# amazon-science/tubelet-transformer

Measured on AMD Instinct MI355X. Metric: clips/sec (TubeR CSN-152 AVA2.1 training step fwd+bwd+clip+AdamW, 32x256x340 clips; whole job), higher is better.
Workload: dtype bf16; 1 GPU; TubeR_CSN152_AVA21 train step, 2 clips/GPU of 3x32x256x340, dropout on, random-init name-hashed weights; global_batch=2, parallelism=dp1, launch_mode=hipgraph, lib_md5=ad1afa292c39

## Files before the change

include/tuber_hip.h:

```cpp
#ifndef TUBER_HIP_H
#define TUBER_HIP_H

#ifdef __cplusplus
extern "C" {
#endif

typedef struct ihipStream_t* hipStream_t;

typedef struct TuberClipDesc {
    long long src_off;
    int H, W;
    int y1, x1, h, w;
    int flip, jitter;
    int hue, sat, val;
    int pad_;
} TuberClipDesc;

int tuber_attn_fwd(const void* Q, const long* mq, const void* K, const long* mk, const void* V, const long* mv, void* O, const long* mo, float* lse, const void* key_padding_mask, int B, int H, int Lq, int Lk, float scale, float pdrop, const void* seed_ptr, unsigned long long salt, hipStream_t stream);

int tuber_attn_bwd(const void* Q, const long* mq, const void* K, const long* mk, const void* V, const long* mv, const void* O, const long* mo, const float* lse, const void* key_padding_mask, const void* dO, const long* mdo, void* dQ, const long* mdq, void* dK, const long* mdk, void* dV, const long* mdv, float* delta, int B, int H, int Lq, int Lk, float scale, float pdrop, const void* seed_ptr, unsigned long long salt, hipStream_t stream);

int tuber_attn_wide_fwd(const void* q, const void* kv, void* o, int NQ, int HW, int T, float pdrop, const void* seed_ptr, unsigned long long salt, hipStream_t stream);

int tuber_attn_wide_bwd(const void* q, const void* kv, const void* dO, void* dq, void* dkv, int NQ, int HW, int T, float pdrop, const void* seed_ptr, unsigned long long salt, hipStream_t stream);
// ... 206 lines not shown

int tuber_ln_bwd_dx_pays(int M, int E_, int Kin);

int tuber_ln_bwd_dx(const void* dy, long lddy, const void* dy2, long lddy2, const void* xhat, const float* rstd, const float* gamma, void* dx, void* dxd, float* partial, int M, int E_, float p, const void* seed_ptr, unsigned long long salt, const void* wt, long ldt, int Kin, void* out, const void* res, const void* cm, float alpha, const void* ga, long ldga, const void* xhat_a, const float* rstd_a, const float* gamma_a, float* partial_a, hipStream_t stream);

int tuber_lsap(const double* cost_in, int nr, int nc, long* row_ind, long* col_ind);

int tuber_stat_rows_reduced(int R);

int tuber_stat_rows_reduce(const float* st0, const float* st1, int R, int C, float* out0, float* out1, hipStream_t stream);

int tuber_bn_finalize(const float* st0, const float* st1, int R, int C, float count, const float* gamma, const float* beta, float* running_mean, float* running_var, long long* num_batches_tracked, float momentum, float eps, float* scale, float* shift, float* mean, float* invstd, hipStream_t stream);

int tuber_bn_finalize_ex(const float* st0, const float* st1, int R, int C, float count, const float* gamma, const float* beta, float* running_mean, float* running_var, long long* num_batches_tracked, float momentum, float eps, float* scale, float* shift, float* mean, float* invstd, hipStream_t stream);

int tuber_bn_count_advance(const long* table, int n, hipStream_t stream);

int tuber_bn_eval_affine(const float* gamma, const float* beta, const float* running_mean, const float* running_var, float eps, float* scale, float* shift, int C, hipStream_t stream);

int tuber_bn_eval_affine_multi(const void* table, int n, int cmax, float eps, hipStream_t stream);

int tuber_bn_frozen_affine_multi(const void* table, int n, int cmax, float eps, hipStream_t stream);

int tuber_bn_frozen_param_grads(const float* st0, const float* st1, int R, int C, const float* mean, const float* invstd, float* dgamma, float* dbeta, hipStream_t stream);

int tuber_bn_bwd_finalize(const float* st0, const float* st1, int R, int C, float count, const float* gamma, const float* mean, const float* invstd, float* cA, float* cB, float* cC, float* dgamma, float* dbeta, int accumulate, hipStream_t stream);

int tuber_block_out_fwd(const void* c4, const float* s4, const float* h4, const void* res, const float* rs, const float* rh, void* y, long M, int C, hipStream_t stream);

int tuber_block_out_fwd_mask(const void* c4, const float* s4, const float* h4, const void* res, const float* rs, const float* rh, void* y, void* ymask, long M, int C, hipStream_t stream);

int tuber_block_out_fwd_f32(const void* c4, const float* s4, const float* h4, const void* res, const float* rs, const float* rh, const float* res32, void* y, float* y32, long M, int C, hipStream_t stream);

int tuber_rowblock_count(long M, int C);

int tuber_block_out_bwd(const void* dy, const void* y, const void* c4, const void* cds, void* dz, float* st_dz, float* st_c4, float* st_ds, long M, int C, hipStream_t stream);

int tuber_bn_bwd_fa_max_rows(void);

int tuber_bn_bwd_fa_rows(long M, int C);

int tuber_bn_bwd_fa_rows_set(int kr);

int tuber_bn_bwd_fa(const float* st0, const float* st1, int R, int C, float count, const float* gamma, const float* mean, const float* invstd, float* dgamma, float* dbeta, const void* dz, const void* x, void* dx, long M, hipStream_t stream);

int tuber_bn_bwd_fa_frozen(const float* st0, const float* st1, int R, int C, const float* gamma, const float* mean, const float* invstd, float* dgamma, float* dbeta, const void* dz, void* dx, long M, hipStream_t stream);

int tuber_bn_bwd_apply(const void* dz, const void* x, const float* cA, const float* cB, const float* cC, void* dx, long M, int C, hipStream_t stream);

int tuber_layernorm_fwd(const void* x, const void* res, const float* gamma, const float* beta, void* y, long ldy, void* xhat, float* rstd, int M, int E, float eps, float p, const void* seed_ptr, unsigned long long salt, hipStream_t stream);

int tuber_layernorm_fwd_f32(const void* x, const float* x32, const void* res, const float* res32, const float* gamma, const float* beta, void* y, long ldy, float* y32, int M, int E, float eps, hipStream_t stream);

int tuber_layernorm_bwd_blocks(int M);

int tuber_layernorm_bwd(const void* dy, long lddy, const void* xhat, const float* rstd, const float* gamma, void* dx, void* dxd, float* partial, float* dgamma, float* dbeta, int accumulate, int M, int E, float p, const void* seed_ptr, unsigned long long salt, hipStream_t stream);

int tuber_reduce_rows(const float* P, float* out, int R, int C, int accumulate, hipStream_t stream);

int tuber_colsum_blocks(long M);

int tuber_colsum(const void* g, float* partial, float* out, int accumulate, long M, int C, long ld, hipStream_t stream);

int tuber_multi_reduce(const void* table, const void* blk, int nblocks, hipStream_t stream);

int tuber_multi_reduce_entry_bytes(void);

int tuber_grad_norm_clip_coef(const float* g, long n, float max_norm, float* partial, float* norm_out, int* step_ptr, hipStream_t stream);

int tuber_adamw_segment(float* p, float* g, float* exp_avg, float* exp_avg_sq, long n, const float* clip, float lr, float beta1, float beta2, float eps, float weight_decay, const int* step_ptr, int write_clipped_grad, const float* hyper, hipStream_t stream);

int tuber_scale_f32(float* x, long n, const float* coef_dev, float coef, hipStream_t stream);

int tuber_rows_dx2(const void* g, long ldg, int M, int N, int Nq, const void* wt, long ldt, int Kin, void* dx, const void* res, void* dpos, hipStream_t stream);

int tuber_stem_pool_fwd(const void* x, const float* sc, const float* sh, void* out, void* arg, int NT, int Hs, int Ws, int Hp, int Wp, hipStream_t stream);

int tuber_stem_pool_bwd_stat_rows(long positions);

int tuber_stem_pool_bwd(const void* gpool, const void* arg, const void* x, const float* sc, const float* sh, void* dz, float* st0, float* st1, int NT, int Hs, int Ws, int Hp, int Wp, hipStream_t stream);

int tuber_stem_conv_blocks(int B, int T, int H, int W);

int tuber_stem_conv_wgrad_blocks(int B, int T, int H, int W);

int tuber_stem_pack_weight(const float* W, void* Wp, hipStream_t stream);

int tuber_stem_conv_fwd(const float* clip, const void* Wp, void* out, float* st0, float* st1, int B, int T, int H, int W, hipStream_t stream);

int tuber_stem_conv_bwd_weight(const float* clip, const void* G, float* partial, float* dW, int accumulate, int B, int T, int H, int W, hipStream_t stream);

int tuber_stem_conv_bwd_weight_bn(const float* clip, const void* dz0, const void* c0, const float* cA, const float* cB, const float* cC, float* partial, float* dW, int accumulate, int B, int T, int H, int W, hipStream_t stream);

int tuber_flag_signal(unsigned* flag, hipStream_t stream);

int tuber_flag_wait(const unsigned* flag, unsigned expect, unsigned* err, hipStream_t stream);


#ifdef __cplusplus
}
#endif
#endif
```

tubelet_transformer_amd/csrc/gen_header.py:

```python
import glob
import os
import re

HERE = os.path.dirname(os.path.abspath(__file__))
ROOT = os.path.dirname(os.path.dirname(HERE))

DOC = {
    "tuber_gemm_nt_addproj": "packed attention in-projection with the positional embedding folded in: C = f(A).B^T + bias with f(A) = A + A2 for the output "
                             "columns [0, add_ncols) (q / k rows of in_proj_weight: with_pos_embed, models/transformer/transformer.py:150-159,215-240) and "
                             "f(A) = A for the v rows -- one GEMM instead of an add kernel and two GEMM launches. add_ncols % 128 == 0.",
    "tuber_bn_bwd_fa": "tuber_bn_bwd_finalize + tuber_bn_bwd_apply in ONE launch for short partial lists (layer3 / layer4 of the CSN body): every workgroup "
                       "derives the coefficients of its 128-channel strip from the R partial rows (fp64) and applies dx = cA*dz + cB*x + cC to its rows; "
                       "dgamma / dbeta accumulated by the first row chunk (NULL: frozen BatchNorm). autograd of nn.BatchNorm3d (ir_CSN_152.py:46,56,64,154).",
    "tuber_bn_bwd_fa_max_rows": "largest R tuber_bn_bwd_fa accepts.",
    "tuber_bn_frozen_affine_multi": "the FROZEN BatchNorm layers of a training-mode forward (nn.BatchNorm3d with module.training == False inside model.train(): "
                                    "F.batch_norm(training=False), models/backbones/ir_CSN_152.py:46,56,64,119,154) in ONE launch over a device table of "
                                    "{gamma, beta, running_mean, running_var, scale, shift, mean, invstd, cA, cB, cC, C} rows: scale / shift bit-identical to "
                                    "tuber_bn_eval_affine, mean = running_mean, invstd = 1 / sqrt(running_var + eps), and the backward coefficients cA = gamma * invstd, "
                                    "cB = cC = 0, so every backward kernel that takes (cA, cB, cC) runs unchanged. The running buffers are not written.",
    "tuber_bn_frozen_param_grads": "dgamma += sum dz * (x - running_mean) * invstd, dbeta += sum dz of a frozen BatchNorm whose affine parameters train (autograd of "
                                   "F.batch_norm(training=False), ir_CSN_152.py:46,56,64,119,154) from the partial rows (sum dz, sum dz*x) of the train-mode path: "
                                   "no count, no coefficient output.",
    "tuber_bn_bwd_fa_frozen": "tuber_bn_bwd_fa for a frozen BatchNorm: dx = gamma * invstd * dz in one launch (autograd of F.batch_norm(training=False), "
                              "ir_CSN_152.py:46,56,64,154); x is not an operand, the partial rows are read only for dgamma / dbeta (NULL: not at all).",
# ... 155 lines not shown
    "tuber_frames_resize": "PIL.Image.resize((nw, nh)) of every decoded frame (datasets/ava_frame.py:146-150; jhmdb_frame.py alike): Pillow's 8-bit two-pass "
                           "fixed-point bicubic (libImaging/Resample.c), packed RGB uint8 [nimg][H][W][3] -> [nimg][Ho][Wo][3], bit-exact.",
    "tuber_clip_prepare": "hflip + crop + ColorJitter + ToTensor/Normalize (datasets/video_transforms.py:69-85,20-66,333-369,308-322; pipeline "
                          "datasets/ava_frame.py:158-176) and the batch collate of utils/misc.py:279-282,367-425 in one pass: uint8 frames -> "
                          "fp32 [N][3][T][Hmax][Wmax] zero padded + bool mask [N][Hmax][Wmax]. One TuberClipDesc per clip (56 bytes: long long src_off; "
                          "int H, W, y1, x1, h, w, flip, jitter, hue, sat, val, pad).",
    "tuber_clip_desc_bytes": "sizeof(TuberClipDesc) as the library was compiled (host-side layout check).",
    "tuber_multi_reduce": "every deferred second-stage reduction of one backward pass in one launch: the weight-gradient launchers called with "
                          "accumulate = 2 (tuber_gemm_tn, tuber_dwconv_*_bwd_weight, tuber_colsum, tuber_layernorm_bwd) leave their partials in place; "
                          "table = MultiReduceEntry[] {const float* P; float* out; long n, stride; int S, mode, C, next}: out[j] += sum_s P[s*stride+j] "
                          "(mode 0 / 2: per element / per float4, s ascending; mode 1: 32-way tree; C > 0: depthwise [S][27][C] -> [C][27]; next: chained contribution to the same out); blk = int2[] (head entry, block in entry), "
                          "1024 / 4096 / 32 elements per block in mode 0 / 2 / 1. Same summation order as the immediate kernels.",
    "tuber_multi_reduce_entry_bytes": "sizeof(MultiReduceEntry) as compiled (host-side layout check).",
    "tuber_temporal_max_fwd": "nn.MaxPool3d((T,1,1)) over the T frames of the backbone features, TEMPORAL_DS_STRATEGY 'max' (models/backbone_builder.py:45-47,73): "
                              "rows (b,t,p) of E bf16 -> rows (b,p) + the uint8 index of the first maximal frame (arg may be NULL in eval).",
    "tuber_temporal_max_bwd": "backward of tuber_temporal_max_fwd: the gradient goes to the frame that held the maximum, zeros elsewhere.",
    "tuber_gemm_nt": "C[M,N] = f(A)[M,K] . B[N,K]^T on MFMA bf16. Replaces every nn.Conv3d(k=1) of the CSN bottlenecks "
                     "(models/backbones/ir_CSN_152.py:41,58,155-161), input_proj/class_proj (models/tuber_ava.py:57-58) and every "
                     "nn.Linear / packed in-projection (models/transformer/transformer.py:159-165,227-245; transformer_layers.py:81-94; "
                     "tuber_ava.py:65-71), plus their data gradients (B = W^T). amode 1 fuses relu(x*a_scale[k]+a_shift[k]) "
                     "(BatchNorm apply, ir_CSN_152.py:72-79) into the A load; gather=1 reads A rows through the strided "
                     "(n,t*st,h*ss,w*ss) map of the down_sample conv (:155-161). epi 0: +bias, +R, ReLU, bf16|fp32 out; "
                     "epi 1: bf16 out + per-column partial (sum, sum^2) rows for training-mode BatchNorm; epi 2: out = acc*[Cm*m_scale+m_shift>0] "
                     "+ partial (sum dz, sum dz*Cm) rows for BatchNorm backward (stat rows optional: with m_scale NULL it is the ReLU / ReLU+Dropout "
                     "backward mask from the saved activation). Accumulators are scaled by alpha first; epi 0 can end with Dropout(drop_p) "
                     "keyed by (seed, salt, m*N+n) -- FFN linear1 (transformer.py:160-162). K % 64 == 0.",
    "tuber_gemm_nt_cfg": "tile configuration tuber_gemm_nt uses for (M,N,K): 13 = 64x64 (two-tile prefetch), 7 = 64x128, 0 = 128x128 (plain epilogue only); 2 / 12 / 17 = rejected A/B variants, built only with -DTUBER_AB_VARIANTS.",
    "tuber_gemm_tn_tile": "output tile edge of the transpose-read weight-gradient kernel for (M, N, K): 128 (mid-M backbone shapes, N and K multiples of 128) or 64.",
    "tuber_gemm_nt_has_cfg": "1 when tuber_gemm_nt_set_cfg(cfg) names a tile configuration this library was built with.",
    "tuber_gemm_nt_stat_rows": "rows of partial statistics tuber_gemm_nt(epi 1|2) writes for (M,N).",
    "tuber_gemm_tn": "dW[N,K] (+)= sum_m G[m,N]^T . f(A)[m,K]: weight gradient of the same convs / linears (autograd of the ops above); "
                     "split over M into fp32 slabs `partial` [tuber_gemm_tn_slabs][N][K], then reduced deterministically.",
    "tuber_gemm_tn_fuses_bias": "can tuber_gemm_tn also produce the bias gradient for this shape: 0 no; 1 yes, accumulated into bias_grad[N] directly (single slab); 2 yes, bias_grad receives one partial row per slab ([tuber_gemm_tn_slabs][N], reduced by the caller).",
    "tuber_gemm_tn_slabs": "number of slabs (size of `partial` / (N*K)) tuber_gemm_tn uses.",
    "tuber_dwconv_fwd": "depthwise Conv3d(C,C,3,groups=C,stride=(st,ss,ss),padding=1) on NDHWC bf16, ResNeXtBottleneck.conv3 "
                        "(ir_CSN_152.py:48-51) with relu(bn1(.)) fused on load (sc/sh may be NULL) and bn3 partial statistics on store.",
    "tuber_dwconv_bwd_data": "input gradient of conv3 fused with the backward of relu(bn1(.)): dz = da*[x*sc+sh>0] + partial (sum dz, sum dz*x).",
    "tuber_dwconv_bwd_weight": "weight gradient of conv3 ([C][27] fp32), activation relu(bn1(x)) recomputed on load.",
    "tuber_dwconv_fwd_stat_rows": "partial-stat rows written by tuber_dwconv_fwd.",
    "tuber_dwconv_bwd_data_stat_rows": "partial-stat rows written by tuber_dwconv_bwd_data.",
    "tuber_dwconv_bwd_weight_blocks": "blocks (size of `partial` / (27*C)) used by tuber_dwconv_bwd_weight.",
    "tuber_dwconv_tile_fwd_bn": "tuber_bn_finalize + tuber_dwconv_tile_fwd in ONE launch: the training-mode BatchNorm in front of conv3 (bn1, ir_CSN_152.py:46-51) is "
                                "finalised inside the conv -- every workgroup derives scale / shift of its 64 channels from the producing conv's R partial rows "
                                "(pst0 = sum x, pst1 = sum x^2 over `count` rows; fp64 sums, the arithmetic of tuber_bn_finalize expression for expression), the first "
                                "workgroup of each channel group writes scale / shift / mean / invstd [C] and updates rmean / rvar / nbt (NULL: none). Other arguments as tuber_dwconv_tile_fwd.",
    "tuber_dwconv_tile_fwd_bn_ex": "tuber_dwconv_tile_fwd_bn with the momentum contract of tuber_bn_finalize_ex: the module's momentum as given, or (momentum < 0) "
                                   "the cumulative average of nn.BatchNorm3d(momentum=None) with nbt read, not written (tuber_bn_count_advance). "
                                   "reference: ir_CSN_152.py:46-51 under torch.optim.swa_utils.update_bn.",
    "tuber_dwconv_tile_fwd": "stride-1 conv3 (ir_CSN_152.py:48-51) with the input planes staged once per workgroup in an LDS ring (activated on the way in): "
                             "same contract as tuber_dwconv_fwd for st = ss = 1; partial-stat rows = tuber_dwconv_tile_blocks.",
    "tuber_dwconv_tile_bwd_data": "LDS-staged data gradient of the stride-1 conv3, fused with the backward of relu(bn1(.)) like tuber_dwconv_bwd_data.",
    "tuber_dwconv_tile_bwd_weight": "LDS-staged weight gradient of the stride-1 conv3 (activation recomputed while staging).",
    "tuber_dwconv_tile_blocks": "workgroups along x of the LDS-staged depthwise kernels = partial-stat rows / weight-gradient partial blocks.",
    "tuber_dwconv_tile_wgrad_blocks": "partial blocks (size of `partial` / (27*C)) of tuber_dwconv_tile_bwd_weight.",
    "tuber_dw_wgrad_reduce": "dw[c][tap] (+)= sum_r partial[r][tap][c]: second stage of the depthwise weight gradient.",
    "tuber_bn_finalize": "training-mode nn.BatchNorm3d(eps=1e-3, momentum=0.1) statistics (ir_CSN_152.py:15-16,46,56,64,119,154): partial rows -> "
                         "mean/invstd, scale=gamma*invstd, shift=beta-mean*scale, running_mean/var (unbiased) and num_batches_tracked update.",
    "tuber_bn_finalize_ex": "tuber_bn_finalize with the module's momentum as given (nn.BatchNorm3d.momentum, ir_CSN_152.py:15-16,46,56,64,119,154; "
                            "running = (1 - m) * running + m * batch, num_batches_tracked += 1). momentum < 0 selects the cumulative average of "
                            "momentum=None (torch.nn.modules.batchnorm._BatchNorm.forward): m = 1 / (n + 1) with n = *num_batches_tracked read on the device, "
                            "which this launch leaves unchanged so that every workgroup sees the same n -- tuber_bn_count_advance increments it after the forward.",
    "tuber_bn_count_advance": "num_batches_tracked += 1 (the `self.num_batches_tracked.add_(1)` of _BatchNorm.forward under momentum=None) for every BatchNorm "
                              "of a DEVICE table of n int64 counter addresses, in ONE launch: the layers finalised in cumulative mode by tuber_bn_finalize_ex / "
                              "tuber_dwconv_tile_fwd_bn_ex during the forward.",
    "tuber_stat_rows_reduce": "first stage for long partial-statistics lists (R > 512 rows: layer1): [R][C] x2 -> [tuber_stat_rows_reduced(R)][C] x2.",
    "tuber_stat_rows_reduced": "rows left by tuber_stat_rows_reduce (R itself when no first stage is needed).",
    "tuber_bn_eval_affine": "eval-mode BatchNorm3d folded to scale/shift from the running statistics.",
    "tuber_bn_bwd_finalize": "BatchNorm backward coefficients: dx = cA*dz + cB*x + cC, dgamma = sum dz*xhat, dbeta = sum dz.",
    "tuber_bn_bwd_apply": "dx = cA*dz + cB*x + cC (BatchNorm backward apply), bf16 [M,C].",
    "tuber_block_out_fwd": "bottleneck join y = relu(bn4(c4) + shortcut) (ir_CSN_152.py:81-90); shortcut = res or bn_ds(res) when rs/rh given.",
    "tuber_block_out_bwd": "backward of the join: dz = dy*[y>0] and the partial statistics of bn4 (and of the down_sample BN).",
    "tuber_rowblock_count": "partial-stat rows written by the row-blocked reduce kernels for M rows.",
    "tuber_layernorm_fwd": "y = LayerNorm(Dropout_p(x) (+ res)) over E in {256, 2048}, eps 1e-5 (nn.LayerNorm, transformer.py:163-167,229-247,116-123; "
                           "transformer_layers.py:84,91,96,437-445); saves xhat (bf16) and rstd for backward.",
    "tuber_layernorm_bwd": "backward of tuber_layernorm_fwd: dx (gradient of res), dxd (gradient of x through the regenerated dropout mask) and dgamma/dbeta via block partials.",
    "tuber_layernorm_bwd_blocks": "blocks used by tuber_layernorm_bwd (partial = 2*blocks*E floats).",
    "tuber_reduce_rows": "out[c] (+)= sum_r P[r][c].",
    "tuber_colsum_blocks": "row blocks (size of `partial` / C) used by tuber_colsum.",
    "tuber_colsum": "bias gradient: out[c] (+)= sum_m g[m][c] for bf16 g.",
    "tuber_gemm_nt_set_cfg": "tuning hook: force tile configuration cfg for every later tuber_gemm_nt (-1 = automatic choice).",
    "tuber_stem_conv_fwd": "stem Conv3d(3,64,(3,7,7),s=(1,2,2),p=(1,3,3)) (ir_CSN_152.py:109-115) as an implicit MFMA GEMM from the fp32 NCDHW clip to NDHWC bf16, "
                           "with the partial statistics of the following BatchNorm; Wp = tuber_stem_pack_weight(conv1.weight).",
    "tuber_stem_conv_bwd_weight": "weight gradient of the stem conv ([64][441] fp32) as an implicit MFMA GEMM (no patch matrix in HBM).",
    "tuber_stem_conv_blocks": "persistent grid size of the stem conv forward = its partial-stat rows.",
    "tuber_stem_conv_wgrad_blocks": "workgroups (= [512][64] fp32 partial slabs) of tuber_stem_conv_bwd_weight.",
    "tuber_stem_pack_weight": "conv1.weight [64][441] fp32 -> [64][512] bf16 with k' = (c,kt,kh)*8 + kw (zero padded).",
    "tuber_stem_pool_fwd": "relu(bn1(.)) + MaxPool3d((1,3,3),s=(1,2,2),p=(0,1,1)) (ir_CSN_152.py:119-122) on NDHWC bf16, C=64; saves the argmax tap.",
    "tuber_stem_pool_bwd": "backward of the pool + relu(bn1(.)): dz and the BN-backward partial statistics.",
    "tuber_stem_pool_bwd_stat_rows": "partial-stat rows written by tuber_stem_pool_bwd.",
    "tuber_attn_fwd": "softmax(scale*QK^T + key_padding_mask)[dropout] V for 32-wide heads, operands read in place through strided token maps "
                      "{ld,sL,s1,s2,B2}: row(l,b) = l*sL + (b/B2)*s1 + (b%B2)*s2. Core of nn.MultiheadAttention "
                      "(transformer.py:159,227,237; tuber_ava.py:138; transformer_layers.py:81,88) and of the hand-rolled MHA (:156-167,306-366).",
    "tuber_attn_bwd": "gradients dQ, dK, dV of tuber_attn_fwd (P recomputed from the saved log-sum-exp).",
    "tuber_attn_wide_fwd": "single-query, 256-wide-head attention of the LSTR pooling decoder (TEMPORAL_DS_STRATEGY decode; "
                           "backbone_builder.py:74-78, transformer_layers.py:156-167,306-366): q [NQ,2048], kv [rows,4096]=[k|v], T<=8 slots per pixel.",
    "tuber_attn_wide_bwd": "gradients dq [NQ,2048] and dkv [rows,4096] of tuber_attn_wide_fwd.",
    "tuber_lsap": "rectangular linear sum assignment on HOST doubles; restates scipy.optimize.linear_sum_assignment (call sites "
                  "models/detr/matcher.py:80, matcher_ucf.py:82) incl. its tie-breaking.",
    "tuber_lsap_device": "the same assignment (scipy.optimize.linear_sum_assignment semantics incl. tie-breaking; matcher.py:80, matcher_ucf.py:82) for all "
                         "(decoder layer, clip) problems at once ON THE DEVICE, one thread per problem: match[l][b][t] = query of target t.",
    "tuber_grad_norm_clip_coef": "global L2 norm of the flat gradient buffer and the clip coefficient min(1, max_norm/(norm+1e-6)), left on the device: "
                                 "torch.nn.utils.clip_grad_norm_(model.parameters(), 0.1) (utils/video_action_recognition.py:153).  A non-finite norm "
                                 "yields coefficient -1 = skip the update and leaves the step count alone: the reference stops BEFORE optimizer.step() on a "
                                 "non-finite loss (video_action_recognition.py:195-198).",
    "tuber_adamw_segment": "AdamW update (torch.optim.AdamW semantics: decoupled decay, bias correction) of one contiguous flat segment with the "
                           "clip coefficient applied to the gradient on the fly (video_action_recognition.py:154; groups train_tuber_ava.py:41-58).",
    "tuber_grad_accum": "gradient accumulation over m micro-batches (DistributedDataParallel's mean over ranks reproduced on fewer GPUs: the mean of "
                        "independent per-rank backward passes, utils/model_utils.py:47-49) over a DEVICE table of nwin [begin, end) int64 windows of the flat "
                        "fp32 gradient buffer, in ONE launch: mode 0 acc = g, mode 1 acc += g, mode 2 g = (acc + g) * scale (scale_dev[0] when given). "
                        "Fixed order: sequential fp32 sum, then one multiply. g and acc 16-byte aligned.",
    "tuber_bn_stats_copy": "snapshot (restore = 0: arena <- buffers) or restore (restore = 1: buffers <- arena) of BatchNorm running statistics "
                           "(running_mean, running_var, num_batches_tracked of nn.BatchNorm3d, models/backbones/ir_CSN_152.py:46,56,64,154) in ONE launch over a "
                           "DEVICE table of nrows {address, arena offset in 32-bit words, words} int64 rows; max_words = the largest row.",
    "tuber_scale_f32": "x *= coef: gradient averaging after the RCCL all-reduce (DistributedDataParallel's mean, utils/model_utils.py:47-49).",
    "tuber_criterion_cost": "Hungarian matching cost C = w_bbox*L1 - w_giou*GIoU - w_class*p of every decoder layer at once, [L,B,Q,Tmax] fp32 "
                            "(HungarianMatcher.forward, models/detr/matcher.py:61-76 / matcher_ucf.py:61-78; generalized_box_iou utils/box_ops.py:41-65).",
    "tuber_criterion_loss": "all loss terms of all layers and their gradients w.r.t. logits / actor logits / boxes in one launch: AVA 3-way weighted CE + "
                            "weighted BCE (models/criterion.py:42-81), JHMDB (C+1)-way CE (:237-262), L1 + GIoU box losses (:97-117).",
    "tuber_cast_f32_bf16": "fp32 -> bf16 copy (bf16 shadow of the fp32 master weights).",
    "tuber_cast_transpose": "W[R][C] fp32 -> W^T[C][ldt] bf16 (B operand of the data-gradient GEMM).",
    "tuber_rows_gather_sum": "out[(a,b,c)] = mul * sum_d in[a*sa+b*sb+c*sc+d*sd] over rows of E bf16: temporal AvgPool3d((4,1,1)) "
                             "(backbone_builder.py:44,73), its backward (broadcast), the x6 replication of src_c (tuber_ava.py:133) and its backward (sum).",
    "tuber_axpby": "out = alpha*a + beta*b (bf16): with_pos_embed adds (transformer.py:150-151), gradient accumulation.",
    "tuber_dropout": "y = keep ? x/(1-p) : 0 with a stateless hash RNG keyed by (seed, index); applying it to a gradient with the same seed is the backward.",
    "tuber_sigmoid_fwd": "boxes = sigmoid(bbox_embed(hs)) (tuber_ava.py:142).",
    "tuber_sigmoid_bwd": "dx = dy*y*(1-y).",
    "tuber_relu_mask": "dx = dy*[h>0] (ReLU backward from the saved activation; FFN and MLP hidden layers).",
    "tuber_multi_transpose_bf16": "every GEMM weight W[R][C] -> W^T[C][ldt] (bf16 shadow of the parameters -> bf16: the B operand of the data-gradient GEMMs, autograd of "
                                  "nn.Conv3d(k=1) / nn.Linear) in one launch over a device table {src_off,dst_off,R,C,ldt,tile_begin,tiles_x,pad} of 64 x 64 tiles.",
    "tuber_cast_pad_rows": "src[R][C] fp32 -> dst[R][ldd] bf16 with zero-filled pad columns (stem 441->448 taps, head gradients).",
    "tuber_rows_scatter_add": "dst[map(m)] += src[m] over the strided (n,t*st,h*ss,w*ss) row map: input gradient of a strided down_sample conv (ir_CSN_152.py:155-161).",
    "tuber_posenc": "PositionEmbeddingSine_3D (models/transformer/position_encoding.py:32-72) of a (B,T,H,W) padding mask, token-major bf16.",
}

HEADER = '''/* tuber_hip.h -- C ABI of libtuber_hip.so: the MI355X (gfx950) kernels behind the TubeR forward/backward path.
 *
 * GENERATED by tubelet_transformer_amd/csrc/gen_header.py from the extern "C" definitions in csrc/*.hip.
 *
 * The reference (amazon-science/tubelet-transformer) has no FFI or operator-plugin boundary: its hot path is stock
 * torch.nn calls (SURVEY.md section 8b).  This ABI is therefore build-defined: one launcher per kernel family, each
 * citing the reference call site(s) whose arithmetic it replaces.  Conventions:
 *   - plain pointers to DEVICE memory + explicit sizes / leading dimensions (in elements); no torch types;
 *   - activations are row-major [rows, channels] bf16 (NDHWC / token-major), master weights and statistics fp32;
 *   - the callee never allocates: outputs, saved tensors and workspaces (`partial`, `st0`, ...) are caller-owned,
 *     sized with the *_rows / *_slabs / *_blocks helper calls;
 *   - every launcher enqueues on `stream` and returns 0, a negative argument-check code (TUBER_EINVAL = -1) or the
 *     positive hipError_t of a failed launch; nothing throws across the ABI.
 */
#ifndef TUBER_HIP_H
#define TUBER_HIP_H

#ifdef __cplusplus
extern "C" {
#endif

typedef struct ihipStream_t* hipStream_t;

/* one clip of tuber_clip_prepare (device memory, 56 bytes) */
typedef struct TuberClipDesc {
    long long src_off;   /* byte offset of the clip's first frame in `frames` (uint8 [T][H][W][3]) */
    int H, W;            /* frame size */
    int y1, x1, h, w;    /* crop window in the (flipped) frame: output (y,x) reads (y1+y, x1+x) */
    int flip, jitter;    /* horizontal flip before the crop; HSV colour jitter on/off */
    int hue, sat, val;   /* ColorJitter shifts (hue in OpenCV half-degrees) */
    int pad_;
} TuberClipDesc;

# ... 50 lines not shown
```

tubelet_transformer_amd/csrc/stem_conv.hip:

```cpp
#include "common.h"

#define SW 64
#define PXW 160
#define KP 512

struct StemGeom { int B, T, H, W, Ho, Wo, tilesW, ntiles; };

struct StemTile { int wt, t, ho, b; long row0; };
__device__ __forceinline__ StemTile stem_tile(const StemGeom& g, int tile) {
    StemTile s;
    s.wt = tile % g.tilesW; int r = tile / g.tilesW;
    s.t = r % g.T; r /= g.T;
    s.ho = r % g.Ho; s.b = r / g.Ho;
    s.row0 = (((long)s.b * g.T + s.t) * g.Ho + s.ho) * g.Wo + s.wt * SW;
    return s;
}
struct StemWalk { int tile, end, step; };
__device__ __forceinline__ StemWalk stem_walk(int ntiles) {
    const int G = gridDim.x;
    if (G & 7) return StemWalk{(int)blockIdx.x, ntiles, G};
    const int chunk = (ntiles + 7) >> 3, x = blockIdx.x & 7, lo = x * chunk;
    return StemWalk{lo + (int)(blockIdx.x >> 3), min(ntiles, lo + chunk), G >> 3};
}
typedef float f32x2u __attribute__((ext_vector_type(2), aligned(4)));
typedef float f32x4u __attribute__((ext_vector_type(4), aligned(4)));

struct StemLane { int l32, half, toff, tkt, tkh; };
__device__ __forceinline__ StemLane stem_lane(const StemGeom& g) {
    StemLane L;
    const int lane = threadIdx.x & 63;
    L.l32 = lane & 31; L.half = lane >> 5;
    const int c = lane / 21, kt = (lane / 7) % 3, kh = lane % 7;
    L.tkt = kt - 1; L.tkh = kh - 3;
    L.toff = ((c * g.T + kt - 1) * g.H + kh - 3) * g.W;
    return L;
}
struct StemMeta { uint32_t kill; int sr, sl, tsr, tsl; };
__device__ __forceinline__ void stem_shift_of(int x0, int W, int& xc, int& sr, int& sl, bool& dead) {
    xc = min(max(x0, 0), W - 4);
    const int d = x0 - xc;
    dead = d >= 4 || d <= -4;
    sr = d > 0 ? 16 * min(d, 3) : 0;
    sl = d < 0 ? 16 * min(-d, 3) : 0;
}
template <int NW> struct StemRuns { int off[64 / NW], dt[64 / NW], dh[64 / NW]; };
template <int NW>
__device__ __forceinline__ StemRuns<NW> stem_runs(const StemGeom& g, int wv) {
    StemRuns<NW> R;
#pragma unroll
    for (int i = 0; i < 64 / NW; ++i) {
        const int r = wv * (64 / NW) + i;
        const int c = r / 21, kt = (r / 7) % 3, kh = r % 7;
        R.dt[i] = r < 63 ? kt - 1 : (1 << 24);
        R.dh[i] = kh - 3;
        R.off[i] = ((c * g.T + kt - 1) * g.H + kh - 3) * g.W;
    }
    return R;
}
template <int NW>
__device__ __forceinline__ void stem_fetch(const float* __restrict__ clip, const StemGeom& g, int tile, const StemLane& L,
                                           const StemRuns<NW>& R, int wv, float4 (&v)[32 / NW + 1], StemMeta& m) {
    constexpr int PAIRS = 32 / NW;
    const StemTile st = stem_tile(g, tile);
    const float* base = clip + (((long)st.b * 3 * g.T + st.t) * g.H + 2 * st.ho) * (long)g.W;
    int xc; bool dead;
    stem_shift_of(128 * st.wt - 3 + 4 * L.l32, g.W, xc, m.sr, m.sl, dead);
    m.kill = dead ? 0x7fffffffu : 0u;
#pragma unroll
    for (int p = 0; p < PAIRS; ++p) {
        int off[2]; bool ok[2];
#pragma unroll
        for (int h = 0; h < 2; ++h) {
            ok[h] = (unsigned)(st.t + R.dt[2 * p + h]) < (unsigned)g.T && (unsigned)(2 * st.ho + R.dh[2 * p + h]) < (unsigned)g.H;
            off[h] = ok[h] ? R.off[2 * p + h] : 0;
        }
        const f32x4u q = *(const f32x4u*)(base + (L.half ? off[1] : off[0]) + xc);
        v[p] = make_float4(q.x, q.y, q.z, q.w);
        if (!(L.half ? ok[1] : ok[0])) m.kill |= 1u << p;
    }
    m.tsr = m.tsl = 0;
    if (wv < 2) {
        const int lane = threadIdx.x & 63;
        int txc; bool tdead;
        stem_shift_of(128 * st.wt - 3 + 4 * (32 + wv), g.W, txc, m.tsr, m.tsl, tdead);
        const bool ok = lane < 63 && (unsigned)(st.t + L.tkt) < (unsigned)g.T && (unsigned)(2 * st.ho + L.tkh) < (unsigned)g.H;
        const f32x4u q = *(const f32x4u*)(base + (ok ? L.toff : 0) + txc);
        v[PAIRS] = make_float4(q.x, q.y, q.z, q.w);
        if (!ok || tdead) m.kill |= 1u << 31;
    }
}
__device__ __forceinline__ uint64_t stem_pack4(const float4& f, int sr, int sl, bool kill) {
    const bf16x4 b = {f2bf(f.x), f2bf(f.y), f2bf(f.z), f2bf(f.w)};
    const uint2 u = as_uint2(b);
    uint64_t w = ((uint64_t)u.y << 32) | u.x;
    w = (w >> sr) << sl;
    return kill ? 0ull : w;
}
template <int NW>
__device__ __forceinline__ void stem_park(bf16 (*P)[PXW], const float4 (&v)[32 / NW + 1], const StemMeta& m, const StemLane& L, int wv) {
    constexpr int PAIRS = 32 / NW;
#pragma unroll
    for (int p = 0; p < PAIRS; ++p)
        *(uint64_t*)&P[wv * (2 * PAIRS) + 2 * p + L.half][4 * L.l32] = stem_pack4(v[p], m.sr, m.sl, (m.kill >> p) & 1);
    if (wv < 2) *(uint64_t*)&P[threadIdx.x & 63][4 * (32 + wv)] = stem_pack4(v[PAIRS], m.tsr, m.tsl, m.kill >> 31);
}
__global__ __launch_bounds__(256, 3) void stem_conv_fwd_kernel(const float* __restrict__ clip, const bf16* __restrict__ Wp,
                                                            bf16* __restrict__ out, float* __restrict__ st0,
                                                            float* __restrict__ st1, StemGeom g) {
    __shared__ __attribute__((aligned(16))) bf16 P[2][64][PXW];
    const int lane = threadIdx.x & 63, wave = threadIdx.x >> 6;
    const int li = lane & 15, gq = lane >> 4;
    bf16x8 wf[16];
#pragma unroll
    for (int ks = 0; ks < 16; ++ks) wf[ks] = as_bf16x8(*(const uint4*)(Wp + (long)(wave * 16 + li) * KP + ks * 32 + gq * 8));
#pragma unroll
    for (int ks = 0; ks < 16; ++ks) asm volatile("" : "+v"(wf[ks]));
    float s0[4] = {0.f, 0.f, 0.f, 0.f}, s1[4] = {0.f, 0.f, 0.f, 0.f};
    float4 pre[9];
    StemMeta meta;
    const StemLane L = stem_lane(g);
    const int wv = __builtin_amdgcn_readfirstlane(wave);
    const StemRuns<4> R = stem_runs<4>(g, wv);
    const StemWalk wk = stem_walk(g.ntiles);
    int tile = wk.tile, buf = 0;
    if (tile < wk.end) {
        stem_fetch<4>(clip, g, tile, L, R, wv, pre, meta);
        stem_park<4>(P[0], pre, meta, L, wv);
    }
    __syncthreads();
    for (; tile < wk.end; tile += wk.step) {
        const int next = tile + wk.step;
        if (next < wk.end) stem_fetch<4>(clip, g, next, L, R, wv, pre, meta);
        f32x4 acc[4];
#pragma unroll
        for (int mt = 0; mt < 4; ++mt) acc[mt] = f32x4{0.f, 0.f, 0.f, 0.f};
#pragma unroll
        for (int ks = 0; ks < 16; ++ks) {
            const int run = ks * 4 + gq;
#pragma unroll
            for (int mt = 0; mt < 4; ++mt) {
                const uint32_t* p = (const uint32_t*)&P[buf][run][2 * (mt * 16 + li)];
                acc[mt] = __builtin_amdgcn_mfma_f32_16x16x32_bf16(wf[ks], as_bf16x8(make_uint4(p[0], p[1], p[2], p[3])), acc[mt], 0, 0, 0);
            }
        }
        if (next < wk.end) stem_park<4>(P[buf ^ 1], pre, meta, L, wv);
        const StemTile st = stem_tile(g, tile);
        const int wt = st.wt;
        const long row0 = st.row0;
#pragma unroll
        for (int mt = 0; mt < 4; ++mt) {
            const int w = wt * SW + mt * 16 + li;
            if (w < g.Wo) {
                bf16x4 o;
#pragma unroll
                for (int r = 0; r < 4; ++r) { o[r] = f2bf(acc[mt][r]); s0[r] += acc[mt][r]; s1[r] += acc[mt][r] * acc[mt][r]; }
                *(uint2*)(out + (row0 + mt * 16 + li) * 64 + wave * 16 + gq * 4) = as_uint2(o);
            }
        }
        __syncthreads();
        buf ^= 1;
    }
    if (st0) {
#pragma unroll
        for (int r = 0; r < 4; ++r) {
            const float a = quad16_sum(s0[r]), b2 = quad16_sum(s1[r]);
            if (li == 0) {
                st0[(long)blockIdx.x * 64 + wave * 16 + gq * 4 + r] = a;
                st1[(long)blockIdx.x * 64 + wave * 16 + gq * 4 + r] = b2;
            }
        }
    }
}

#define EOW 72
#define WG_THREADS 512
__device__ __forceinline__ void stem_park_eo(bf16 (*PE)[EOW], bf16 (*PO)[EOW], const float4 (&v)[5], const StemMeta& m, const StemLane& L, int wv) {
    auto put = [&](int r, int q, uint64_t w) {
        const uint32_t lo = (uint32_t)w, hi = (uint32_t)(w >> 32);
        *(uint32_t*)&PE[r][2 * q] = __builtin_amdgcn_perm(hi, lo, 0x05040100);
        *(uint32_t*)&PO[r][2 * q] = __builtin_amdgcn_perm(hi, lo, 0x07060302);
    };
#pragma unroll
    for (int p = 0; p < 4; ++p) put(wv * 8 + 2 * p + L.half, L.l32, stem_pack4(v[p], m.sr, m.sl, (m.kill >> p) & 1));
    if (wv < 2) put(threadIdx.x & 63, 32 + wv, stem_pack4(v[4], m.tsr, m.tsl, m.kill >> 31));
}
__device__ __forceinline__ bf16x8 stem_frag_shift(const bf16* row, int m0, int s) {
    const uint4 a = *(const uint4*)(row + m0);
    const uint2 b = *(const uint2*)(row + m0 + 8);
    uint32_t w[6] = {a.x, a.y, a.z, a.w, b.x, b.y};
    uint4 o;
    if (s & 2) { w[0] = w[1]; w[1] = w[2]; w[2] = w[3]; w[3] = w[4]; w[4] = w[5]; }
    if (s & 1) {
        o.x = __builtin_amdgcn_alignbit(w[1], w[0], 16); o.y = __builtin_amdgcn_alignbit(w[2], w[1], 16);
        o.z = __builtin_amdgcn_alignbit(w[3], w[2], 16); o.w = __builtin_amdgcn_alignbit(w[4], w[3], 16);
    } else {
        o = make_uint4(w[0], w[1], w[2], w[3]);
    }
    return as_bf16x8(o);
}

template <int MINW, bool BNG>
__global__ __launch_bounds__(WG_THREADS, MINW) void stem_conv_bwd_w_kernel(const float* __restrict__ clip, const bf16* __restrict__ G,
                                                                       const bf16* __restrict__ X, const float* __restrict__ cA,
                                                                       const float* __restrict__ cB, const float* __restrict__ cC,
                                                                       float* __restrict__ partial, StemGeom g) {
    __shared__ __attribute__((aligned(16))) bf16 PE[64][EOW];
    __shared__ __attribute__((aligned(16))) bf16 PO[64][EOW];
    __shared__ __attribute__((aligned(16))) bf16 GT[64][72];
    __shared__ __attribute__((aligned(16))) float COEF[3][64];
    if (BNG && threadIdx.x < 64) { COEF[0][threadIdx.x] = cA[threadIdx.x]; COEF[1][threadIdx.x] = cB[threadIdx.x]; COEF[2][threadIdx.x] = cC[threadIdx.x]; }
    const int lane = threadIdx.x & 63, wave = threadIdx.x >> 6;
    const int li = lane & 15, gq = lane >> 4;
    f32x4 acc[7][2];
#pragma unroll
    for (int a = 0; a < 7; ++a)
#pragma unroll
        for (int b = 0; b < 2; ++b) acc[a][b] = f32x4{0.f, 0.f, 0.f, 0.f};
    const int ci = (lane & 3) | ((lane >> 4) << 2), mi = ((lane >> 2) & 3) + 4 * wave;
    float4 pre[5];
    StemMeta meta;
    uint2 gr[2], gx[2];
    const StemLane L = stem_lane(g);
    const int wv = __builtin_amdgcn_readfirstlane(wave);
    const int nh = wv >> 2, rb = wv & 3;
    const StemRuns<8> R = stem_runs<8>(g, wv);
    auto fetch = [&](int tile) {
        stem_fetch<8>(clip, g, tile, L, R, wv, pre, meta);
        const StemTile st = stem_tile(g, tile);
#pragma unroll
        for (int j = 0; j < 2; ++j) {
            const int w = st.wt * SW + mi * 2 + j;
            gr[j] = w < g.Wo ? *(const uint2*)(G + (st.row0 + mi * 2 + j) * 64 + ci * 4) : make_uint2(0, 0);
            if (BNG) gx[j] = w < g.Wo ? *(const uint2*)(X + (st.row0 + mi * 2 + j) * 64 + ci * 4) : make_uint2(0, 0);
        }
    };
    const StemWalk wk = stem_walk(g.ntiles);
    if (wk.tile < wk.end) fetch(wk.tile);
    for (int tile = wk.tile; tile < wk.end; tile += wk.step) {
        __syncthreads();
        stem_park_eo(PE, PO, pre, meta, L, wv);
        {
            bf16x4 x0 = as_bf16x4(gr[0]), x1 = as_bf16x4(gr[1]);
            if (BNG) {
                const StemTile st = stem_tile(g, tile);
                const bool ok0 = st.wt * SW + mi * 2 < g.Wo, ok1 = st.wt * SW + mi * 2 + 1 < g.Wo;
                const float4 a = *(const float4*)&COEF[0][ci * 4], b = *(const float4*)&COEF[1][ci * 4], c = *(const float4*)&COEF[2][ci * 4];
                const float av[4] = {a.x, a.y, a.z, a.w}, bv[4] = {b.x, b.y, b.z, b.w}, cv[4] = {c.x, c.y, c.z, c.w};
                const bf16x4 y0 = as_bf16x4(gx[0]), y1 = as_bf16x4(gx[1]);
#pragma unroll
                for (int q = 0; q < 4; ++q) {
                    x0[q] = ok0 ? f2bf(fmaf(av[q], bf2f(x0[q]), fmaf(bv[q], bf2f(y0[q]), cv[q]))) : (bf16)0.f;
                    x1[q] = ok1 ? f2bf(fmaf(av[q], bf2f(x1[q]), fmaf(bv[q], bf2f(y1[q]), cv[q]))) : (bf16)0.f;
                }
            }
#pragma unroll
            for (int c = 0; c < 4; ++c) *(bf16x2*)&GT[ci * 4 + c][mi * 2] = bf16x2{x0[c], x1[c]};
        }
        if (tile + wk.step < wk.end) fetch(tile + wk.step);
        __syncthreads();
#pragma unroll
        for (int ms = 0; ms < 2; ++ms) {
            bf16x8 gb[2];
#pragma unroll
            for (int nt = 0; nt < 2; ++nt) gb[nt] = as_bf16x8(*(const uint4*)&GT[(nh * 2 + nt) * 16 + li][ms * 32 + gq * 8]);
#pragma unroll
            for (int kw = 0; kw < 7; ++kw) {
                const int kt = kw;
                const bf16* row = (kw & 1) ? &PO[rb * 16 + li][0] : &PE[rb * 16 + li][0];
                const bf16x8 pa = stem_frag_shift(row, ms * 32 + gq * 8, kw >> 1);
#pragma unroll
                for (int nt = 0; nt < 2; ++nt) acc[kt][nt] = __builtin_amdgcn_mfma_f32_16x16x32_bf16(pa, gb[nt], acc[kt][nt], 0, 0, 0);
            }
        }
    }
    float* o = partial + (long)blockIdx.x * KP * 64;
#pragma unroll
    for (int kt = 0; kt < 7; ++kt) {
        const int kw = kt;
#pragma unroll
        for (int nt = 0; nt < 2; ++nt)
#pragma unroll
            for (int r = 0; r < 4; ++r)
                o[(long)((rb * 16 + gq * 4 + r) * 8 + kw) * 64 + (nh * 2 + nt) * 16 + li] = acc[kt][nt][r];
    }
}

__global__ void stem_pack_w_kernel(const float* __restrict__ W, bf16* __restrict__ Wp) {
    const int i = blockIdx.x * blockDim.x + threadIdx.x;
    if (i >= 64 * KP) return;
    const int n = i / KP, kp = i % KP, run = kp >> 3, kw = kp & 7;
    Wp[i] = (run < 63 && kw < 7) ? f2bf(W[n * 441 + run * 7 + kw]) : (bf16)0.f;
}
__global__ __launch_bounds__(1024) void stem_wgrad_reduce_kernel(const float* __restrict__ partial, float* __restrict__ dW, int nwg, int accumulate) {
    __shared__ float red[32][33];
    const int cl = threadIdx.x & 31, rg = threadIdx.x >> 5;
    const int i = blockIdx.x * 32 + cl;
    float a = 0.f;
    for (int s = rg; s < nwg; s += 32) a += partial[(long)s * KP * 64 + i];
    red[rg][cl] = a;
    __syncthreads();
    if (rg == 0) {
        a = 0.f;
#pragma unroll
        for (int k = 0; k < 32; ++k) a += red[k][cl];
        const int kp = i / 64, n = i % 64, run = kp >> 3, kw = kp & 7;
        if (run < 63 && kw < 7) {
            float* o = dW + n * 441 + run * 7 + kw;
            *o = accumulate ? *o + a : a;
        }
    }
}

static StemGeom stem_geom(int B, int T, int H, int W) {
    StemGeom g;
    g.B = B; g.T = T; g.H = H; g.W = W;
    g.Ho = (H + 6 - 7) / 2 + 1; g.Wo = (W + 6 - 7) / 2 + 1;
    g.tilesW = (g.Wo + SW - 1) / SW;
    g.ntiles = B * T * g.Ho * g.tilesW;
    return g;
}

extern "C" {

int tuber_stem_conv_blocks(int B, int T, int H, int W) {
    constexpr int cap = 768;
    const StemGeom g = stem_geom(B, T, H, W);
    return g.ntiles < cap ? g.ntiles : cap;
}
int tuber_stem_conv_wgrad_blocks(int B, int T, int H, int W) {
    constexpr int cap = 256;
    const StemGeom g = stem_geom(B, T, H, W);
    return g.ntiles < cap ? g.ntiles : cap;
}

int tuber_stem_pack_weight(const float* W, void* Wp, hipStream_t stream) {
    hipLaunchKernelGGL(stem_pack_w_kernel, dim3(64 * KP / 256), dim3(256), 0, stream, W, (bf16*)Wp);
    TUBER_RETURN_LAUNCH();
}

int tuber_stem_conv_fwd(const float* clip, const void* Wp, void* out, float* st0, float* st1, int B, int T, int H, int W,
                        hipStream_t stream) {
    if (B <= 0 || T <= 0 || H < 7 || W < 7) return TUBER_EINVAL;
    const StemGeom g = stem_geom(B, T, H, W);
    hipLaunchKernelGGL(stem_conv_fwd_kernel, dim3(tuber_stem_conv_blocks(B, T, H, W)), dim3(256), 0, stream, clip, (const bf16*)Wp,
                       (bf16*)out, st0, st1, g);
    TUBER_RETURN_LAUNCH();
}

int tuber_stem_conv_bwd_weight(const float* clip, const void* G, float* partial, float* dW, int accumulate, int B, int T, int H, int W,
                               hipStream_t stream) {
    if (B <= 0 || T <= 0 || H < 7 || W < 7) return TUBER_EINVAL;
    const StemGeom g = stem_geom(B, T, H, W);
    const int nwg = tuber_stem_conv_wgrad_blocks(B, T, H, W);
    if (nwg > 256) hipLaunchKernelGGL((stem_conv_bwd_w_kernel<4, false>), dim3(nwg), dim3(WG_THREADS), 0, stream, clip, (const bf16*)G, nullptr, nullptr, nullptr, nullptr, partial, g);
    else hipLaunchKernelGGL((stem_conv_bwd_w_kernel<2, false>), dim3(nwg), dim3(WG_THREADS), 0, stream, clip, (const bf16*)G, nullptr, nullptr, nullptr, nullptr, partial, g);
    hipLaunchKernelGGL(stem_wgrad_reduce_kernel, dim3(KP * 64 / 32), dim3(1024), 0, stream, partial, dW, nwg, accumulate);
    TUBER_RETURN_LAUNCH();
}

int tuber_stem_conv_bwd_weight_bn(const float* clip, const void* dz0, const void* c0, const float* cA, const float* cB, const float* cC,
                                  float* partial, float* dW, int accumulate, int B, int T, int H, int W, hipStream_t stream) {
    if (B <= 0 || T <= 0 || H < 7 || W < 7 || !dz0 || !c0 || !cA || !cB || !cC) return TUBER_EINVAL;
    const StemGeom g = stem_geom(B, T, H, W);
    const int nwg = tuber_stem_conv_wgrad_blocks(B, T, H, W);
    if (nwg > 256) hipLaunchKernelGGL((stem_conv_bwd_w_kernel<4, true>), dim3(nwg), dim3(WG_THREADS), 0, stream, clip, (const bf16*)dz0, (const bf16*)c0, cA, cB, cC, partial, g);
    else hipLaunchKernelGGL((stem_conv_bwd_w_kernel<2, true>), dim3(nwg), dim3(WG_THREADS), 0, stream, clip, (const bf16*)dz0, (const bf16*)c0, cA, cB, cC, partial, g);
    hipLaunchKernelGGL(stem_wgrad_reduce_kernel, dim3(KP * 64 / 32), dim3(1024), 0, stream, partial, dW, nwg, accumulate);
    TUBER_RETURN_LAUNCH();
}

}
```

Baseline: 146.8 clips/s.

## Retile stem conv forward to 32x32 wave tiles with a smaller persistent grid

The stem conv forward now gives each wave a 32-channel by 32-column tile, so each weight fragment is reused across two column tiles. It also drops occupancy to 2 waves per SIMD and caps the grid at 512 workgroups, with unused stat rows zero-filled. Tile coordinates advance incrementally instead of using divisions each iteration, in both the forward and weight-grad kernels. The old kernel stays available behind a test hook, but the added register pressure and lower occupancy may limit the gain on a small part of the step.

Result: no change. 147.1 clips/s (median of 4 runs) (+0.2%).

```diff
diff --git a/include/tuber_hip.h b/include/tuber_hip.h
--- a/include/tuber_hip.h
+++ b/include/tuber_hip.h
@@ -312,6 +312,8 @@
 
 int tuber_stem_conv_blocks(int B, int T, int H, int W);
 
+int tuber_stem_conv_variant_set(int variant, int grid_cap);
+
 int tuber_stem_conv_wgrad_blocks(int B, int T, int H, int W);
 
 int tuber_stem_pack_weight(const float* W, void* Wp, hipStream_t stream);
diff --git a/tubelet_transformer_amd/csrc/gen_header.py b/tubelet_transformer_amd/csrc/gen_header.py
--- a/tubelet_transformer_amd/csrc/gen_header.py
+++ b/tubelet_transformer_amd/csrc/gen_header.py
@@ -261,7 +261,13 @@
     "tuber_stem_conv_fwd": "stem Conv3d(3,64,(3,7,7),s=(1,2,2),p=(1,3,3)) (ir_CSN_152.py:109-115) as an implicit MFMA GEMM from the fp32 NCDHW clip to NDHWC bf16, "
                            "with the partial statistics of the following BatchNorm; Wp = tuber_stem_pack_weight(conv1.weight).",
     "tuber_stem_conv_bwd_weight": "weight gradient of the stem conv ([64][441] fp32) as an implicit MFMA GEMM (no patch matrix in HBM).",
-    "tuber_stem_conv_blocks": "persistent grid size of the stem conv forward = its partial-stat rows.",
+    "tuber_stem_conv_blocks": "partial-statistics ROWS of the stem conv forward: st0 / st1 are [rows][64] and this is the R of the tuber_stat_rows_reduce / "
+                              "tuber_bn_finalize* call that consumes them. Not the grid: the kernel launches at most this many workgroups, workgroup b writes "
+                              "its sums to row b, and rows without an owning workgroup are written as zeros by the kernel, so all rows are defined and their sum "
+                              "is the statistic.",
+    "tuber_stem_conv_variant_set": "test hook: variant 0 = the forward's 32-channel x 32-column wave tiles (default), 1 = the 16-channel x 64-column kernel it "
+                                   "replaced (bit-identical output; kept for the parity test and A/B timing); grid_cap > 0 bounds the forward's grid so that "
+                                   "small shapes cycle the persistent loop, 0 = no bound.",
     "tuber_stem_conv_wgrad_blocks": "workgroups (= [512][64] fp32 partial slabs) of tuber_stem_conv_bwd_weight.",
     "tuber_stem_pack_weight": "conv1.weight [64][441] fp32 -> [64][512] bf16 with k' = (c,kt,kh)*8 + kw (zero padded).",
     "tuber_stem_pool_fwd": "relu(bn1(.)) + MaxPool3d((1,3,3),s=(1,2,2),p=(0,1,1)) (ir_CSN_152.py:119-122) on NDHWC bf16, C=64; saves the argmax tap.",
diff --git a/tubelet_transformer_amd/csrc/stem_conv.hip b/tubelet_transformer_amd/csrc/stem_conv.hip
--- a/tubelet_transformer_amd/csrc/stem_conv.hip
+++ b/tubelet_transformer_amd/csrc/stem_conv.hip
@@ -12,6 +12,14 @@
     s.wt = tile % g.tilesW; int r = tile / g.tilesW;
     s.t = r % g.T; r /= g.T;
     s.ho = r % g.Ho; s.b = r / g.Ho;
+    s.row0 = (((long)s.b * g.T + s.t) * g.Ho + s.ho) * g.Wo + s.wt * SW;
+    return s;
+}
+__device__ __forceinline__ StemTile stem_tile_add(const StemGeom& g, StemTile s, const StemTile& d) {
+    s.wt += d.wt; int c = s.wt >= g.tilesW; s.wt -= c ? g.tilesW : 0;
+    s.t += d.t + c; c = s.t >= g.T; s.t -= c ? g.T : 0;
+    s.ho += d.ho + c; c = s.ho >= g.Ho; s.ho -= c ? g.Ho : 0;
+    s.b += d.b + c;
     s.row0 = (((long)s.b * g.T + s.t) * g.Ho + s.ho) * g.Wo + s.wt * SW;
     return s;
 }
@@ -58,10 +66,9 @@
     return R;
 }
 template <int NW>
-__device__ __forceinline__ void stem_fetch(const float* __restrict__ clip, const StemGeom& g, int tile, const StemLane& L,
+__device__ __forceinline__ void stem_fetch(const float* __restrict__ clip, const StemGeom& g, const StemTile& st, const StemLane& L,
                                            const StemRuns<NW>& R, int wv, float4 (&v)[32 / NW + 1], StemMeta& m) {
     constexpr int PAIRS = 32 / NW;
-    const StemTile st = stem_tile(g, tile);
     const float* base = clip + (((long)st.b * 3 * g.T + st.t) * g.H + 2 * st.ho) * (long)g.W;
     int xc; bool dead;
     stem_shift_of(128 * st.wt - 3 + 4 * L.l32, g.W, xc, m.sr, m.sl, dead);
@@ -104,9 +111,13 @@
         *(uint64_t*)&P[wv * (2 * PAIRS) + 2 * p + L.half][4 * L.l32] = stem_pack4(v[p], m.sr, m.sl, (m.kill >> p) & 1);
     if (wv < 2) *(uint64_t*)&P[threadIdx.x & 63][4 * (32 + wv)] = stem_pack4(v[PAIRS], m.tsr, m.tsl, m.kill >> 31);
 }
-__global__ __launch_bounds__(256, 3) void stem_conv_fwd_kernel(const float* __restrict__ clip, const bf16* __restrict__ Wp,
-                                                            bf16* __restrict__ out, float* __restrict__ st0,
-                                                            float* __restrict__ st1, StemGeom g) {
+__device__ __forceinline__ void stem_zero_rows(float* __restrict__ st0, float* __restrict__ st1, int nrows) {
+    if (threadIdx.x < 64)
+        for (long r = (long)blockIdx.x + gridDim.x; r < nrows; r += gridDim.x) st0[r * 64 + threadIdx.x] = st1[r * 64 + threadIdx.x] = 0.f;
+}
+__global__ __launch_bounds__(256, 3) void stem_conv_fwd16_kernel(const float* __restrict__ clip, const bf16* __restrict__ Wp,
+                                                              bf16* __restrict__ out, float* __restrict__ st0,
+                                                              float* __restrict__ st1, int nrows, StemGeom g) {
     __shared__ __attribute__((aligned(16))) bf16 P[2][64][PXW];
     const int lane = threadIdx.x & 63, wave = threadIdx.x >> 6;
     const int li = lane & 15, gq = lane >> 4;
@@ -123,14 +134,17 @@
     const StemRuns<4> R = stem_runs<4>(g, wv);
     const StemWalk wk = stem_walk(g.ntiles);
     int tile = wk.tile, buf = 0;
+    const StemTile dstep = stem_tile(g, wk.step);
+    StemTile st = stem_tile(g, tile);
     if (tile < wk.end) {
-        stem_fetch<4>(clip, g, tile, L, R, wv, pre, meta);
+        stem_fetch<4>(clip, g, st, L, R, wv, pre, meta);
         stem_park<4>(P[0], pre, meta, L, wv);
     }
     __syncthreads();
     for (; tile < wk.end; tile += wk.step) {
         const int next = tile + wk.step;
-        if (next < wk.end) stem_fetch<4>(clip, g, next, L, R, wv, pre, meta);
+        const StemTile nx = stem_tile_add(g, st, dstep);
+        if (next < wk.end) stem_fetch<4>(clip, g, nx, L, R, wv, pre, meta);
         f32x4 acc[4];
 #pragma unroll
         for (int mt = 0; mt < 4; ++mt) acc[mt] = f32x4{0.f, 0.f, 0.f, 0.f};
@@ -144,7 +158,6 @@
             }
         }
         if (next < wk.end) stem_park<4>(P[buf ^ 1], pre, meta, L, wv);
-        const StemTile st = stem_tile(g, tile);
         const int wt = st.wt;
         const long row0 = st.row0;
 #pragma unroll
@@ -159,6 +172,7 @@
         }
         __syncthreads();
         buf ^= 1;
+        st = nx;
     }
     if (st0) {
 #pragma unroll
@@ -169,6 +183,110 @@
                 st1[(long)blockIdx.x * 64 + wave * 16 + gq * 4 + r] = b2;
             }
         }
+        stem_zero_rows(st0, st1, nrows);
+    }
+}
+
+template <int NM>
+__device__ __forceinline__ void stem_fwd_mma(const bf16 (*Pb)[PXW], const bf16x8 (&wf)[2][16], int gq, int col, f32x4 (&acc)[2][2]) {
+#pragma unroll
+    for (int ks = 0; ks < 16; ++ks) {
+        const int run = ks * 4 + gq;
+#pragma unroll
+        for (int mt = 0; mt < NM; ++mt) {
+            const uint32_t* p = (const uint32_t*)&Pb[run][2 * (col + mt * 16)];
+            const bf16x8 pf = as_bf16x8(make_uint4(p[0], p[1], p[2], p[3]));
+#pragma unroll
+            for (int ct = 0; ct < 2; ++ct) acc[ct][mt] = __builtin_amdgcn_mfma_f32_16x16x32_bf16(wf[ct][ks], pf, acc[ct][mt], 0, 0, 0);
+        }
+    }
+}
+__global__ __launch_bounds__(256, 2) void stem_conv_fwd_kernel(const float* __restrict__ clip, const bf16* __restrict__ Wp,
+                                                            bf16* __restrict__ out, float* __restrict__ st0,
+                                                            float* __restrict__ st1, int nrows, StemGeom g) {
+    __shared__ __attribute__((aligned(16))) bf16 P[2][64][PXW];
+    const int lane = threadIdx.x & 63, wave = threadIdx.x >> 6;
+    const int li = lane & 15, gq = lane >> 4;
+    const int wv = __builtin_amdgcn_readfirstlane(wave);
+    const int ch = wv & 1, cw = wv >> 1;
+    bf16x8 wf[2][16];
+#pragma unroll
+    for (int ct = 0; ct < 2; ++ct)
+#pragma unroll
+        for (int ks = 0; ks < 16; ++ks) wf[ct][ks] = as_bf16x8(*(const uint4*)(Wp + (long)(ch * 32 + ct * 16 + li) * KP + ks * 32 + gq * 8));
+#pragma unroll
+    for (int ct = 0; ct < 2; ++ct)
+#pragma unroll
+        for (int ks = 0; ks < 16; ++ks) asm volatile("" : "+v"(wf[ct][ks]));
+    float s0[2][4], s1[2][4];
+#pragma unroll
+    for (int ct = 0; ct < 2; ++ct)
+#pragma unroll
+        for (int r = 0; r < 4; ++r) s0[ct][r] = s1[ct][r] = 0.f;
+    float4 pre[9];
+    StemMeta meta;
+    const StemLane L = stem_lane(g);
+    const StemRuns<4> R = stem_runs<4>(g, wv);
+    const StemWalk wk = stem_walk(g.ntiles);
+    int tile = wk.tile, buf = 0;
+    const StemTile dstep = stem_tile(g, wk.step);
+    StemTile st = stem_tile(g, tile);
+    if (tile < wk.end) {
+        stem_fetch<4>(clip, g, st, L, R, wv, pre, meta);
+        stem_park<4>(P[0], pre, meta, L, wv);
+    }
+    __syncthreads();
+    for (; tile < wk.end; tile += wk.step) {
+        const int next = tile + wk.step;
+        const StemTile nx = stem_tile_add(g, st, dstep);
+        if (next < wk.end) stem_fetch<4>(clip, g, nx, L, R, wv, pre, meta);
+        const int live = g.Wo - st.wt * SW - cw * 32;
+        f32x4 acc[2][2];
+#pragma unroll
+        for (int ct = 0; ct < 2; ++ct)
+#pragma unroll
+            for (int mt = 0; mt < 2; ++mt) acc[ct][mt] = f32x4{0.f, 0.f, 0.f, 0.f};
+        if (live > 16) stem_fwd_mma<2>(P[buf], wf, gq, cw * 32 + li, acc);
+        else if (live > 0) stem_fwd_mma<1>(P[buf], wf, gq, cw * 32 + li, acc);
+        if (next < wk.end) stem_park<4>(P[buf ^ 1], pre, meta, L, wv);
+#pragma unroll
+        for (int mt = 0; mt < 2; ++mt) {
+            if (mt * 16 + li < live) {
+#pragma unroll
+                for (int ct = 0; ct < 2; ++ct) {
+                    bf16x4 o;
+#pragma unroll
+                    for (int r = 0; r < 4; ++r) { o[r] = f2bf(acc[ct][mt][r]); s0[ct][r] += acc[ct][mt][r]; s1[ct][r] += acc[ct][mt][r] * acc[ct][mt][r]; }
+                    *(uint2*)(out + (st.row0 + cw * 32 + mt * 16 + li) * 64 + ch * 32 + ct * 16 + gq * 4) = as_uint2(o);
+                }
+            }
+        }
+        __syncthreads();
+        buf ^= 1;
+        st = nx;
+    }
+    if (st0) {
+        float* red = (float*)&P[0][0][0];
+#pragma unroll
+        for (int ct = 0; ct < 2; ++ct)
+#pragma unroll
+            for (int r = 0; r < 4; ++r) {
+                s0[ct][r] = quad16_sum(s0[ct][r]);
+                s1[ct][r] = quad16_sum(s1[ct][r]);
+                if (cw == 1 && li == 0) { red[ch * 32 + ct * 16 + gq * 4 + r] = s0[ct][r]; red[64 + ch * 32 + ct * 16 + gq * 4 + r] = s1[ct][r]; }
+            }
+        __syncthreads();
+        if (cw == 0 && li == 0) {
+#pragma unroll
+            for (int ct = 0; ct < 2; ++ct)
+#pragma unroll
+                for (int r = 0; r < 4; ++r) {
+                    const int c = ch * 32 + ct * 16 + gq * 4 + r;
+                    st0[(long)blockIdx.x * 64 + c] = s0[ct][r] + red[c];
+                    st1[(long)blockIdx.x * 64 + c] = s1[ct][r] + red[64 + c];
+                }
+        }
+        stem_zero_rows(st0, st1, nrows);
     }
 }
 
@@ -224,9 +342,8 @@
     const int wv = __builtin_amdgcn_readfirstlane(wave);
     const int nh = wv >> 2, rb = wv & 3;
     const StemRuns<8> R = stem_runs<8>(g, wv);
-    auto fetch = [&](int tile) {
-        stem_fetch<8>(clip, g, tile, L, R, wv, pre, meta);
-        const StemTile st = stem_tile(g, tile);
+    auto fetch = [&](const StemTile& st) {
+        stem_fetch<8>(clip, g, st, L, R, wv, pre, meta);
 #pragma unroll
         for (int j = 0; j < 2; ++j) {
             const int w = st.wt * SW + mi * 2 + j;
@@ -235,14 +352,15 @@
         }
     };
     const StemWalk wk = stem_walk(g.ntiles);
-    if (wk.tile < wk.end) fetch(wk.tile);
+    const StemTile dstep = stem_tile(g, wk.step);
+    StemTile st = stem_tile(g, wk.tile);
+    if (wk.tile < wk.end) fetch(st);
     for (int tile = wk.tile; tile < wk.end; tile += wk.step) {
         __syncthreads();
         stem_park_eo(PE, PO, pre, meta, L, wv);
         {
             bf16x4 x0 = as_bf16x4(gr[0]), x1 = as_bf16x4(gr[1]);
             if (BNG) {
-                const StemTile st = stem_tile(g, tile);
                 const bool ok0 = st.wt * SW + mi * 2 < g.Wo, ok1 = st.wt * SW + mi * 2 + 1 < g.Wo;
                 const float4 a = *(const float4*)&COEF[0][ci * 4], b = *(const float4*)&COEF[1][ci * 4], c = *(const float4*)&COEF[2][ci * 4];
                 const float av[4] = {a.x, a.y, a.z, a.w}, bv[4] = {b.x, b.y, b.z, b.w}, cv[4] = {c.x, c.y, c.z, c.w};
@@ -256,7 +374,9 @@
 #pragma unroll
             for (int c = 0; c < 4; ++c) *(bf16x2*)&GT[ci * 4 + c][mi * 2] = bf16x2{x0[c], x1[c]};
         }
-        if (tile + wk.step < wk.end) fetch(tile + wk.step);
+        const int wt = st.wt;
+        st = stem_tile_add(g, st, dstep);
+        if (tile + wk.step < wk.end) fetch(st);
         __syncthreads();
 #pragma unroll
         for (int ms = 0; ms < 2; ++ms) {
@@ -327,6 +447,17 @@
     const StemGeom g = stem_geom(B, T, H, W);
     return g.ntiles < cap ? g.ntiles : cap;
 }
+static int g_stem_variant = 0, g_stem_grid_cap = 0;
+int tuber_stem_conv_variant_set(int variant, int grid_cap) {
+    if ((variant != 0 && variant != 1) || grid_cap < 0) return TUBER_EINVAL;
+    g_stem_variant = variant; g_stem_grid_cap = grid_cap;
+    return 0;
+}
+static int stem_fwd_grid(const StemGeom& g) {
+    int cap = g_stem_variant == 1 ? 768 : 512;
+    if (g_stem_grid_cap > 0 && g_stem_grid_cap < cap) cap = g_stem_grid_cap;
+    return g.ntiles < cap ? g.ntiles : cap;
+}
 int tuber_stem_conv_wgrad_blocks(int B, int T, int H, int W) {
     constexpr int cap = 256;
     const StemGeom g = stem_geom(B, T, H, W);
@@ -342,8 +473,9 @@
                         hipStream_t stream) {
     if (B <= 0 || T <= 0 || H < 7 || W < 7) return TUBER_EINVAL;
     const StemGeom g = stem_geom(B, T, H, W);
-    hipLaunchKernelGGL(stem_conv_fwd_kernel, dim3(tuber_stem_conv_blocks(B, T, H, W)), dim3(256), 0, stream, clip, (const bf16*)Wp,
-                       (bf16*)out, st0, st1, g);
+    const int rows = tuber_stem_conv_blocks(B, T, H, W);
+    if (g_stem_variant == 1) hipLaunchKernelGGL(stem_conv_fwd16_kernel, dim3(stem_fwd_grid(g)), dim3(256), 0, stream, clip, (const bf16*)Wp, (bf16*)out, st0, st1, rows, g);
+    else hipLaunchKernelGGL(stem_conv_fwd_kernel, dim3(stem_fwd_grid(g)), dim3(256), 0, stream, clip, (const bf16*)Wp, (bf16*)out, st0, st1, rows, g);
     TUBER_RETURN_LAUNCH();
 }
 
```
